# JonasGeiping/fullbatchtraining

Measured on AMD Instinct MI355X. Metric: full-batch GD images/sec (ResNet-18 CIFAR-10 shaped, all chunks accumulated per step), higher is better.
Workload: dtype bf16

## Files before the change

fullbatchtraining_amd/csrc/conv_igemm.hip:

```cpp
#include "common.h"
#include "profile.h"

#include "conv_params.h"

template <typename T, int BN_CO>
__global__ __launch_bounds__(256) void conv_igemm_kernel(const ConvParams p) {
    constexpr int EB = ET<T>::EB;
    constexpr int BKE = 128 / EB;
    constexpr int WROWS = BN_CO / 32;
    constexpr int FI = BN_CO / 32;
    constexpr int FJ = 4;
    constexpr int TILE_CHUNKS = (128 + BN_CO) * 8;
    __shared__ uint4 lds[2 * TILE_CHUNKS];

    const int tid = threadIdx.x, lane = tid & 63, wave = tid >> 6;
    const int wave_co = wave >> 1, wave_px = wave & 1;
    const int mblk = blockIdx.x, co_blk = blockIdx.y, cls = blockIdx.z;
    const int cpy = (p.os == 2) ? (cls >> 1) : 0, cpx = (p.os == 2) ? (cls & 1) : 0;
    const int chunk = tid & 7, lrow = tid >> 3;

    int a_img[4], a_y[4], a_x[4];
    const int qHW = p.qH * p.qW;
#pragma unroll
    for (int i = 0; i < 4; ++i) {
        const int m = mblk * 128 + lrow + 32 * i;
        if (m < p.M) {
            const int n = m / qHW, rem = m - n * qHW, qy = rem / p.qW, qx = rem - qy * p.qW;
            a_img[i] = n * p.Hs * p.Ws; a_y[i] = qy * p.ss; a_x[i] = qx * p.ss;
        } else {
            a_img[i] = 0; a_y[i] = -(1 << 28); a_x[i] = 0;
        }
    }
    const int first_img = (mblk * 128) / qHW;
    const char* wbase = p.wgt + (long long)(first_img / p.imgs_per_wset) * p.wset_stride_bytes;
    const int taps = p.R * p.S;
    const long long wrow_bytes = (long long)taps * p.Cs * EB;
    const char* wptr[WROWS];
#pragma unroll
    for (int i = 0; i < WROWS; ++i) wptr[i] = wbase + (long long)(co_blk * BN_CO + lrow + 32 * i) * wrow_bytes + chunk * 16;

    auto tap_valid = [&](int t, int& dy, int& dx) -> bool {
        const int r = t / p.S, s = t - r * p.S;
        if (p.mode == 0) { dy = r - p.pad; dx = s - p.pad; return true; }
        if (p.os == 1) { dy = p.pad - r; dx = p.pad - s; return true; }
        const int vy = cpy + p.pad - r, vx = cpx + p.pad - s;
        if ((vy & 1) || (vx & 1)) return false;
        dy = vy >> 1; dx = vx >> 1;
        return true;
    };
    const int kc = (p.Cs + BKE - 1) / BKE;
    int n_valid = 0;
    for (int t = 0; t < taps; ++t) { int dy, dx; n_valid += tap_valid(t, dy, dx) ? 1 : 0; }
    const int n_iter = n_valid * kc;

    uint4 ra[4], rw[WROWS];
    int cur_t = -1, cur_c = kc, cur_dy = 0, cur_dx = 0;
    auto advance = [&]() {
        if (++cur_c >= kc) {
            cur_c = 0;
            do { ++cur_t; } while (cur_t < taps && !tap_valid(cur_t, cur_dy, cur_dx));
        }
    };
    auto gload = [&]() {
        const int c0 = cur_c * BKE;
        const bool cvalid = c0 + chunk * ET<T>::VEC < p.Cs;
#pragma unroll
        for (int i = 0; i < 4; ++i) {
            const int sy = a_y[i] + cur_dy, sx = a_x[i] + cur_dx;
            const bool ok = cvalid && (unsigned)sy < (unsigned)p.Hs && (unsigned)sx < (unsigned)p.Ws;
            ra[i] = make_uint4(0, 0, 0, 0);
            if (ok) ra[i] = *(const uint4*)(p.src + ((long long)(a_img[i] + sy * p.Ws + sx) * p.Cs + c0) * EB + chunk * 16);
        }
#pragma unroll
        for (int i = 0; i < WROWS; ++i) {
            rw[i] = make_uint4(0, 0, 0, 0);
            if (cvalid) rw[i] = *(const uint4*)(wptr[i] + ((long long)cur_t * p.Cs + c0) * EB);
        }
    };
    auto lstore = [&](int buf) {
        uint4* base = lds + buf * TILE_CHUNKS;
#pragma unroll
        for (int i = 0; i < 4; ++i) { const int row = lrow + 32 * i; base[row * 8 + (chunk ^ (row & 7))] = ra[i]; }
#pragma unroll
        for (int i = 0; i < WROWS; ++i) { const int row = 128 + lrow + 32 * i; base[row * 8 + (chunk ^ (row & 7))] = rw[i]; }
    };

    f32x4_t acc[FI][FJ];
#pragma unroll
    for (int i = 0; i < FI; ++i)
#pragma unroll
        for (int j = 0; j < FJ; ++j) acc[i][j] = (f32x4_t){0.f, 0.f, 0.f, 0.f};

    if (n_iter > 0) {
        advance(); gload(); lstore(0);
        __syncthreads();
        for (int it = 0; it < n_iter; ++it) {
            const int buf = it & 1;
            const bool more = it + 1 < n_iter;
            if (more) { advance(); gload(); }
            const uint4* base = lds + buf * TILE_CHUNKS;
#pragma unroll
            for (int h = 0; h < 2; ++h) {
                const int pc = ((lane >> 4) + 4 * h) ^ (lane & 7);
                uint4 wf[FI], pf[FJ];
#pragma unroll
                for (int i = 0; i < FI; ++i) wf[i] = base[(128 + wave_co * (BN_CO / 2) + i * 16 + (lane & 15)) * 8 + pc];
#pragma unroll
                for (int j = 0; j < FJ; ++j) pf[j] = base[(wave_px * 64 + j * 16 + (lane & 15)) * 8 + pc];
#pragma unroll
                for (int i = 0; i < FI; ++i)
#pragma unroll
                    for (int j = 0; j < FJ; ++j) acc[i][j] = mma_chunk<T>(wf[i], pf[j], acc[i][j]);
            }
            if (more) lstore(buf ^ 1);
            __syncthreads();
        }
    }

    float ssum[FI][4], ssq[FI][4];
#pragma unroll
    for (int i = 0; i < FI; ++i)
#pragma unroll
        for (int r = 0; r < 4; ++r) { ssum[i][r] = 0.f; ssq[i][r] = 0.f; }
#pragma unroll
    for (int j = 0; j < FJ; ++j) {
        const int m = mblk * 128 + wave_px * 64 + j * 16 + (lane & 15);
        if (m < p.M) {
            const int n = m / qHW, rem = m - n * qHW, qy = rem / p.qW, qx = rem - qy * p.qW;
            const int oy = qy * p.os + cpy, ox = qx * p.os + cpx;
            const long long pix = ((long long)n * p.Hd + oy) * p.Wd + ox;
#pragma unroll
            for (int i = 0; i < FI; ++i) {
                const int co = co_blk * BN_CO + wave_co * (BN_CO / 2) + i * 16 + (lane >> 4) * 4;
                float v[4] = {acc[i][j][0], acc[i][j][1], acc[i][j][2], acc[i][j][3]};
                if (p.addend_mode == 1) {
                    const char* ap = p.addend + (pix * p.Cd + co) * EB;
                    if constexpr (EB == 4) { const float4 a = *(const float4*)ap; v[0] += a.x; v[1] += a.y; v[2] += a.z; v[3] += a.w; }
                    else { const uint2 a = *(const uint2*)ap; v[0] += __uint_as_float(a.x << 16); v[1] += __uint_as_float(a.x & 0xffff0000u);
                           v[2] += __uint_as_float(a.y << 16); v[3] += __uint_as_float(a.y & 0xffff0000u); }
                } else if (p.addend_mode == 2) {
                    const long long apix = ((long long)n * (p.Hd >> 1) + (oy >> 1)) * (p.Wd >> 1) + (ox >> 1);
                    const char* ap = p.addend + (apix * p.Cd + co) * EB;
                    if constexpr (EB == 4) { const float4 a = *(const float4*)ap; v[0] += 0.25f * a.x; v[1] += 0.25f * a.y; v[2] += 0.25f * a.z; v[3] += 0.25f * a.w; }
                    else { const uint2 a = *(const uint2*)ap; v[0] += 0.25f * __uint_as_float(a.x << 16); v[1] += 0.25f * __uint_as_float(a.x & 0xffff0000u);
                           v[2] += 0.25f * __uint_as_float(a.y << 16); v[3] += 0.25f * __uint_as_float(a.y & 0xffff0000u); }
                }
                char* dp = p.dst + (pix * p.Cd + co) * EB;
                if constexpr (EB == 4) *(float4*)dp = make_float4(v[0], v[1], v[2], v[3]);
                else *(uint2*)dp = make_uint2(pack_bf16x2(v[0], v[1]), pack_bf16x2(v[2], v[3]));
#pragma unroll
                for (int r = 0; r < 4; ++r) { ssum[i][r] += v[r]; ssq[i][r] += v[r] * v[r]; }
            }
        }
    }
    if (p.stat != nullptr) {
        float* red = (float*)lds;
        __syncthreads();
#pragma unroll
        for (int i = 0; i < FI; ++i)
#pragma unroll
            for (int r = 0; r < 4; ++r) {
                float a = ssum[i][r], b = ssq[i][r];
                a = row16_sum(a); b = row16_sum(b);
                if ((lane & 15) == 0) {
                    const int col = wave_co * (BN_CO / 2) + i * 16 + (lane >> 4) * 4 + r;
                    red[(wave_px * BN_CO + col) * 2] = a; red[(wave_px * BN_CO + col) * 2 + 1] = b;
                }
            }
        __syncthreads();
        if (tid < BN_CO) {
            const float a = red[tid * 2] + red[(BN_CO + tid) * 2];
            const float b = red[tid * 2 + 1] + red[(BN_CO + tid) * 2 + 1];
            const long long blk = (long long)cls * gridDim.x + mblk;
            p.stat[blk * p.Cd + co_blk * BN_CO + tid] = a;
            p.stat[((long long)p.n_mblocks + blk) * p.Cd + co_blk * BN_CO + tid] = b;
        }
    }
}

int fb_try_conv3x3_halo4(const fb_conv_args* a, hipStream_t st);
int fb_try_conv3x3_halo5(const fb_conv_args* a, hipStream_t st);
int fb_conv3x3_halo5_takes(const fb_conv_args* a);
int fb_try_conv3x3s2_dgrad_quad(const fb_conv_args* a, hipStream_t st);
int fb_try_conv1x1_k32(const fb_conv_args* a, hipStream_t st);
int fb_try_conv1x1_stream(const fb_conv_args* a, hipStream_t st);
int fb_try_conv1x1_gemm(const fb_conv_args* a, hipStream_t st);
int fb_try_conv1x1_pipe(const fb_conv_args* a, hipStream_t st);

int fb_conv1x1_pipe_takes(const fb_conv_args* a);
int fb_conv3x3_halo4_takes(const fb_conv_args* a);
int fb_conv1x1_gemm_takes(const fb_conv_args* a);
static int igemm_masked_addend_ok(const fb_conv_args* a) {
    if (getenv("FB_IGEMM_NO_MASK") != nullptr || a->mode != 1 || a->stride != 1 || a->bst_x) return 0;
    if (a->Cs % 32 != 0 || a->Cd % 64 != 0) return 0;
    static const bool v1 = getenv("FB_IGEMM_V1") != nullptr;
    if (v1) return 0;
    ConvParams p{};
    p.n_img = a->n_img; p.Hs = a->Hs; p.Ws = a->Ws; p.Cs = a->Cs; p.Hd = a->Hd; p.Wd = a->Wd; p.Cd = a->Cd; p.R = a->R; p.S = a->S;
    p.qH = a->Hd; p.qW = a->Wd;
    return fb_igemm_glds_fits(p, a->dtype);
}
extern "C" int32_t fb_conv_masked_addend_supported(const fb_conv_args* a) {
    if (!a || !a->addend || !a->addend_mask || a->addend_mode != 1) return 0;
    return fb_conv3x3_halo5_takes(a) || fb_conv1x1_pipe_takes(a) || fb_conv3x3_halo4_takes(a) || fb_conv1x1_gemm_takes(a) || igemm_masked_addend_ok(a);
}

extern "C" int32_t fb_conv_bwd_stat_supported(const fb_conv_args* a) {
    static const bool disabled = getenv("FB_DISABLE_FUSED_BWD_STAT") != nullptr;
    if (disabled || !a || !a->bst_x || !a->bst_mask || !a->stat_partial || a->mode != 1 || a->dtype != FB_BF16) return 0;
    if ((long long)a->n_img * a->Hd * a->Wd % 128 != 0) return 0;
    static const char* widths = getenv("FB_FUSED_BWD_STAT_W");
    if (widths) {
        char tag[8];
        snprintf(tag, sizeof(tag), "%d,", a->Wd);
        char list[64];
        snprintf(list, sizeof(list), "%s,", widths);
        if (!strstr(list, tag) || (a->Wd < 10 && list != strstr(list, tag) && *(strstr(list, tag) - 1) != ',')) return 0;
    }
    return fb_conv3x3_halo5_takes(a) || fb_conv3x3_halo4_takes(a);
}

template <typename T> static int launch_conv(const ConvParams& p, int classes, hipStream_t st) {
    const int mblocks = (p.M + 127) / 128;
    if (p.Cd % 128 == 0 && (long long)mblocks * (p.Cd / 128) * classes >= 512) {
        dim3 grid(mblocks, p.Cd / 128, classes);
        hipLaunchKernelGGL((conv_igemm_kernel<T, 128>), grid, dim3(256), 0, st, p);
    } else {
        dim3 grid(mblocks, p.Cd / 64, classes);
        hipLaunchKernelGGL((conv_igemm_kernel<T, 64>), grid, dim3(256), 0, st, p);
    }
    return 0;
}

extern "C" int fb_conv2d(const fb_conv_args* a, void* stream) {
    if (!a || !a->src || !a->wgt || !a->dst) FB_FAIL(FB_ERR_ARG, "fb_conv2d: null pointer");
    const int EB = a->dtype == FB_F32 ? 4 : 2;
    if (a->Cs % 32 != 0) FB_FAIL(FB_ERR_SHAPE, "fb_conv2d: Cs=%d must be a multiple of 32", a->Cs);
    if (a->Cd % 64 != 0) FB_FAIL(FB_ERR_SHAPE, "fb_conv2d: Cd=%d must be a multiple of 64", a->Cd);
    if (a->mode != 0 && a->mode != 1) FB_FAIL(FB_ERR_ARG, "fb_conv2d: mode %d", a->mode);
    if (a->addend_mask && !fb_conv_masked_addend_supported(a))
        FB_FAIL(FB_ERR_UNSUPPORTED, "fb_conv2d: addend_mask is not implemented for this shape (ask fb_conv_masked_addend_supported)");
    if (a->bst_x && !fb_conv_bwd_stat_supported(a))
        FB_FAIL(FB_ERR_UNSUPPORTED, "fb_conv2d: the fused BatchNorm-backward reduction is not implemented for this shape (ask fb_conv_bwd_stat_supported)");
    if (a->stride != 1 && a->stride != 2) FB_FAIL(FB_ERR_UNSUPPORTED, "fb_conv2d: stride %d", a->stride);
    ConvParams p;
    p.src = (const char*)a->src; p.wgt = (const char*)a->wgt; p.dst = (char*)a->dst; p.addend = (const char*)a->addend;
    p.stat = a->stat_partial;
    p.n_img = a->n_img; p.Hs = a->Hs; p.Ws = a->Ws; p.Cs = a->Cs; p.Hd = a->Hd; p.Wd = a->Wd; p.Cd = a->Cd;
    p.R = a->R; p.S = a->S; p.stride = a->stride; p.pad = a->pad; p.mode = a->mode;
    p.imgs_per_wset = a->imgs_per_wset > 0 ? a->imgs_per_wset : a->n_img;
    p.wset_stride_bytes = a->wset_stride * EB;
    p.addend_mode = a->addend ? a->addend_mode : 0;
    p.addend_mask = a->addend ? (const unsigned char*)a->addend_mask : nullptr;
    p.amax_src = a->dtype == FB_F32 ? a->amax_src : nullptr; p.amax_wgt = a->dtype == FB_F32 ? a->amax_wgt : nullptr;
    if ((p.amax_src == nullptr) != (p.amax_wgt == nullptr)) FB_FAIL(FB_ERR_ARG, "fb_conv2d: amax_src and amax_wgt go together");
    p.amax_imgs = a->amax_imgs > 0 ? a->amax_imgs : a->n_img;
    int classes = 1;
    if (a->mode == 0) {
        if (a->Hd != (a->Hs + 2 * a->pad - a->R) / a->stride + 1 || a->Wd != (a->Ws + 2 * a->pad - a->S) / a->stride + 1)
            FB_FAIL(FB_ERR_SHAPE, "fb_conv2d: fwd output %dx%d inconsistent with input %dx%d", a->Hd, a->Wd, a->Hs, a->Ws);
        p.qH = a->Hd; p.qW = a->Wd; p.os = 1; p.ss = a->stride;
    } else {
        if (a->Hs != (a->Hd + 2 * a->pad - a->R) / a->stride + 1 || a->Ws != (a->Wd + 2 * a->pad - a->S) / a->stride + 1)
            FB_FAIL(FB_ERR_SHAPE, "fb_conv2d: dgrad shapes inconsistent");
        if (a->stat_partial && !a->bst_x) FB_FAIL(FB_ERR_ARG, "fb_conv2d: statistics in mode 1 need bst_x / bst_mask");
        if (a->stride == 1) { p.qH = a->Hd; p.qW = a->Wd; p.os = 1; }
        else {
            if ((a->Hd & 1) || (a->Wd & 1)) FB_FAIL(FB_ERR_SHAPE, "fb_conv2d: stride-2 dgrad needs even input dims");
            p.qH = a->Hd / 2; p.qW = a->Wd / 2; p.os = 2; classes = 4;
        }
        p.ss = 1;
    }
    p.M = a->n_img * p.qH * p.qW;
    p.n_mblocks = ((p.M + 127) / 128) * classes;
    hipStream_t st = (hipStream_t)stream;
    const int32_t info[FB_PROF_INFO] = {a->n_img, a->Hs, a->Ws, a->Cs, a->Hd, a->Wd, a->Cd, a->R, a->stride,
                                        (a->addend ? a->addend_mode : 0) | (a->addend_mask ? 4 : 0) | (a->bst_x ? 8 : 0) | (a->dtype << 4), 0};
    const int prof = fb_prof_begin(a->mode == 0 ? FB_PROF_IGEMM_FWD : FB_PROF_IGEMM_DGRAD, st, info);
    static const bool v1 = getenv("FB_IGEMM_V1") != nullptr;
    int kernel = 0;
    if (fb_try_conv1x1_k32(a, st)) kernel = FB_K_CONV1X1_K32;
    else if ((a->mode == 0 || a->addend) && (a->Cs == 256 || a->Cs == 128) && fb_try_conv1x1_gemm(a, st)) kernel = FB_K_CONV1X1_GEMM;
    else if (fb_try_conv1x1_pipe(a, st)) kernel = FB_K_CONV1X1_PIPE;
    else if (fb_try_conv1x1_stream(a, st)) kernel = FB_K_CONV1X1_STREAM;
    else if (fb_try_conv1x1_gemm(a, st)) kernel = FB_K_CONV1X1_GEMM;
    else if (fb_try_conv3x3s2_dgrad_quad(a, st)) kernel = FB_K_S2_DGRAD_QUAD;
    else if (fb_try_conv3x3_halo5(a, st)) kernel = FB_K_HALO5;
    else if (fb_try_conv3x3_halo4(a, st)) kernel = FB_K_HALO4;
    else {
        p.zeros = nullptr;
        kernel = FB_K_IGEMM_GLDS;
        if (v1 || !fb_launch_igemm_glds(p, classes, a->dtype, st)) {
            if (p.addend_mask) FB_FAIL(FB_ERR_UNSUPPORTED, "fb_conv2d: the register-staged implicit GEMM does not apply addend_mask (tensor beyond 2^31 bytes per tile or FB_IGEMM_V1)");
            if (p.amax_src) FB_FAIL(FB_ERR_UNSUPPORTED, "fb_conv2d: the register-staged implicit GEMM has no fp16x2 path (tensor beyond 2^31 bytes or FB_IGEMM_V1)");
            if (a->dtype == FB_F32) launch_conv<float>(p, classes, st); else launch_conv<bf16_tag>(p, classes, st);
            kernel = FB_K_IGEMM_V1;
        }
    }
    fb_prof_kernel(prof, kernel);
    fb_prof_end(prof, st);
    FB_CHECK_LAUNCH("fb_conv2d");
    return FB_OK;
}
```

fullbatchtraining_amd/lib.py:

```python
import ctypes as C
import os
import struct

import torch

FB_F32, FB_BF16 = 0, 1
EXPECTED_ABI = 17
_LIB_PATH = os.environ.get("FB_LIB_PATH") or os.path.join(os.path.dirname(os.path.abspath(__file__)), "csrc", "libfbengine.so")

c_void_p, c_int, c_i64, c_float, c_double = C.c_void_p, C.c_int32, C.c_int64, C.c_float, C.c_double


class ConvArgs(C.Structure):
    _fields_ = [("src", c_void_p), ("wgt", c_void_p), ("dst", c_void_p), ("addend", c_void_p), ("stat_partial", c_void_p),
                ("n_img", c_int), ("Hs", c_int), ("Ws", c_int), ("Cs", c_int), ("Hd", c_int), ("Wd", c_int), ("Cd", c_int),
                ("R", c_int), ("S", c_int), ("stride", c_int), ("pad", c_int), ("mode", c_int),
                ("imgs_per_wset", c_int), ("wset_stride", c_i64), ("addend_mode", c_int), ("dtype", c_int), ("addend_mask", c_void_p),
                ("bst_x", c_void_p), ("bst_mask", c_void_p), ("amax_src", c_void_p), ("amax_wgt", c_void_p), ("amax_imgs", c_int)]


class WgradArgs(C.Structure):
    _fields_ = [("x", c_void_p), ("dy", c_void_p), ("dw_partial", c_void_p),
                ("n_img", c_int), ("Hs", c_int), ("Ws", c_int), ("Cs", c_int), ("Hd", c_int), ("Wd", c_int), ("Cd", c_int),
                ("R", c_int), ("S", c_int), ("stride", c_int), ("pad", c_int),
                ("imgs_per_group", c_int), ("split_k", c_int), ("dtype", c_int), ("group_stride", c_i64), ("amax_x", c_void_p), ("amax_dy", c_void_p),
                ("bn_x", c_void_p), ("bn_mask", c_void_p), ("bn_coef", c_void_p)]


_CTYPES = {"v": None, "i": c_int, "l": c_i64, "f": c_float, "d": c_double, "p": c_void_p, "s": C.c_char_p,
           "C": C.POINTER(ConvArgs), "W": C.POINTER(WgradArgs)}
PROF_CLASSES = ("igemm_fwd", "igemm_dgrad", "wgrad", "bn_apply", "bn_bwd_reduce", "bn_bwd_apply")
PROF_KERNELS = {0: "?", 1: "conv_igemm_kernel (register-staged)", 2: "conv_igemm_v3_kernel", 3: "conv3x3s1_halo4_kernel", 4: "conv3x3s1_c64_halo5_kernel",
                5: "conv3x3s2_dgrad_quad_kernel", 6: "conv1x1_k32_kernel", 7: "conv1x1_stream_kernel", 8: "conv3x3s2_fwd_kernel", 9: "conv1x1_pipe_kernel", 10: "conv1x1_gemm_kernel",
                16: "conv_wgrad_kernel", 17: "conv_wgrad3x3_kernel", 18: "conv_wgrad3x3_v2_kernel", 19: "conv_wgrad1x1_kernel"}
_FROM_LIBRARY = ("EXPORTS", "_SIGS", "_ARG_CODES", "MT_BLOCKS", "PROF_INFO")


def __getattr__(name):
    if name in _FROM_LIBRARY:
        load()
        return globals()[name]
    raise AttributeError(f"module {__name__!r} has no attribute {name!r}")


def profile_enable(on, capacity=32768):
    lib = load()
    if lib.fb_profile_enable(1 if on else 0, capacity) != 0:
        raise EngineError(lib.fb_last_error_string().decode())


def profile_read():
    lib = load()
    k = len(PROF_CLASSES)
    ms, n, d = (c_double * k)(), (c_i64 * k)(), (c_i64 * k)()
    if lib.fb_profile_read(ms, n, d) != 0:
        raise EngineError(lib.fb_last_error_string().decode())
    return {k: (ms[i], n[i], d[i]) for i, k in enumerate(PROF_CLASSES)}


def profile_read_launches(cap=1 << 18):
    lib = load()
    info, ms = (c_int * (cap * (PROF_INFO + 1)))(), (c_float * cap)()
    n = lib.fb_profile_read_launches(info, ms, cap)
    if n < 0:
        raise EngineError(lib.fb_last_error_string().decode())
    w = PROF_INFO + 1
    return [(PROF_CLASSES[info[i * w]], tuple(info[i * w + 1:(i + 1) * w]), ms[i]) for i in range(n)]


_lib = None


class EngineError(RuntimeError):
    pass


def check_layout(cls, fields, size):
    mine, end = cls._fields_, 0
    for i, (name, offset, nbytes, code) in enumerate(fields):
        if offset != -(-end // nbytes) * nbytes:
            raise EngineError(f"{cls.__name__}: the library's field {name} at offset {offset} does not follow its predecessor, which ends at {end}")
        end = offset + nbytes
        if i >= len(mine) or mine[i][0] != name:
            raise EngineError(f"{cls.__name__}: field {i} is {name} in the library, {mine[i][0] if i < len(mine) else 'missing'} here")
        here = getattr(cls, name)
        if (here.offset, here.size) != (offset, nbytes) or mine[i][1] is not _CTYPES[code]:
            raise EngineError(f"{cls.__name__}.{name}: {mine[i][1].__name__} of {here.size} bytes at offset {here.offset} here, "
                              f"'{code}' of {nbytes} bytes at offset {offset} in the library")
    if len(mine) > len(fields):
        raise EngineError(f"{cls.__name__}: field {mine[len(fields)][0]} is not in the library's struct")
    if C.sizeof(cls) != size:
        raise EngineError(f"{cls.__name__}: {C.sizeof(cls)} bytes here, {size} in the library")


def _struct_fields(lib, which):
    name, offset, nbytes, code = C.c_char_p(), c_int(), c_int(), C.c_char()
    out = []
    while len(out) < lib.fb_struct_field(which, len(out), C.byref(name), C.byref(offset), C.byref(nbytes), C.byref(code)):
        out.append((name.value.decode(), offset.value, nbytes.value, code.value.decode()))
    return out


def load():
    global _lib, EXPORTS, _SIGS, _ARG_CODES, MT_BLOCKS, PROF_INFO
    if _lib is None:
        if not os.path.isfile(_LIB_PATH):
            raise EngineError(f"{_LIB_PATH} is missing: run `python -m fullbatchtraining_amd.build` (needs hipcc). "
                              "The engine has no CPU or PyTorch fallback.")
        lib = C.CDLL(_LIB_PATH)
        if lib.fb_abi_version() != EXPECTED_ABI:
            raise EngineError(f"{_LIB_PATH} has ABI version {lib.fb_abi_version()}, this package expects {EXPECTED_ABI}: rebuild it with "
                              "`python -m fullbatchtraining_amd.build --force`")
        lib.fb_entry_name.restype = lib.fb_entry_sig.restype = C.c_char_p
        exports, sigs, codes = [], {}, {}
        for i in range(lib.fb_entry_count()):
            name, sig = lib.fb_entry_name(i).decode(), lib.fb_entry_sig(i).decode()
            fn, argtypes = getattr(lib, name), [_CTYPES[c] for c in sig[2:]]
            fn.restype, fn.argtypes = _CTYPES[sig[0]], argtypes
            exports.append(name)
            if lib.fb_entry_kind(i) > 0:
                sigs[name], codes[name] = argtypes, sig[2:]
        for which, cls in enumerate((ConvArgs, WgradArgs)):
            check_layout(cls, _struct_fields(lib, which), lib.fb_struct_size(which))
        if lib.fb_abi_constant(b"FB_PROF_CLASSES") != len(PROF_CLASSES):
            raise EngineError(f"the library times {lib.fb_abi_constant(b'FB_PROF_CLASSES')} kernel classes, PROF_CLASSES names {len(PROF_CLASSES)}")
        EXPORTS, _SIGS, _ARG_CODES = tuple(exports), sigs, codes
        MT_BLOCKS, PROF_INFO = lib.fb_abi_constant(b"FB_MT_BLOCKS"), lib.fb_abi_constant(b"FB_PROF_INFO")
        _lib = lib
    return _lib


def _ptr(t):
    if t is None:
        return None
    if isinstance(t, int):
        return t
    return t.data_ptr()


def _stream():
    return torch.cuda.current_stream().cuda_stream


def call(name, *args):
    lib = load()
    st = _stream()
    status = getattr(lib, name)(*args, st)
    if status != 0:
        raise EngineError(f"{name} failed ({status}): {lib.fb_last_error_string().decode()} [args: {args}]")
    if _recorder is not None:
        _recorder.add_call(name, args, st)


_recorder = None


def recording():
    return _recorder is not None


def current_recorder():
    return _recorder


def _check(status, what):
    if status != 0:
        raise EngineError(f"{what} failed ({status}): {load().fb_last_error_string().decode()}")


def event_new():
    ev = load().fb_event_new()
    if ev < 0:
        raise EngineError(load().fb_last_error_string().decode())
    return ev


def event_count():
    return int(load().fb_event_count())


def event_record(ev, stream=None):
    st = _stream() if stream is None else stream.cuda_stream
    _check(load().fb_event_record(ev, st), "fb_event_record")
    if _recorder is not None:
        _recorder.add_event(1, ev, st)


def event_wait(ev, stream=None):
    st = _stream() if stream is None else stream.cuda_stream
    _check(load().fb_event_wait(ev, st), "fb_event_wait")
    if _recorder is not None:
        _recorder.add_event(2, ev, st)


def _pack_words(name, args):
    load()
    sig = _ARG_CODES[name][:-1]
    if len(args) != len(sig):
        raise EngineError(f"{name}: {len(args)} arguments for a signature of {len(sig)}")
    words = (C.c_uint64 * len(sig))()
    blob = None
    for i, (code, a) in enumerate(zip(sig, args)):
        if code == "f":
            words[i] = struct.unpack("<I", struct.pack("<f", float(a)))[0]
        elif code == "d":
            words[i] = struct.unpack("<Q", struct.pack("<d", float(a)))[0]
        elif code in "pil":
            words[i] = (0 if a is None else int(a)) & 0xFFFFFFFFFFFFFFFF
        elif i == 0 and code in "CW" and hasattr(a, "_obj"):
            blob = a._obj
        else:
            raise EngineError(f"{name}: argument {i} of type '{code}' cannot be recorded")
    return words, blob


class CommandList:

    def __init__(self, handle, n_streams, keep, events=()):
        self.handle, self.n_streams, self.keep, self.events = handle, n_streams, keep, list(events)
        self.used_streams = frozenset()

    def __len__(self):
        return int(load().fb_cmdlist_size(self.handle))

    def replay(self, streams):
        if any(s is None and i in self.used_streams for i, s in enumerate(streams)):
            raise EngineError("CommandList.replay: the list has commands for a stream index that is None now")
        arr = (c_void_p * self.n_streams)(*[None if s is None else s.cuda_stream for s in streams])
        _check(load().fb_cmdlist_replay(self.handle, arr, self.n_streams), "fb_cmdlist_replay")

    def __del__(self):
        try:
            if self.handle and _lib is not None:
                _lib.fb_cmdlist_destroy(self.handle)
        except Exception:
            pass
        self.handle = None


class Recorder:

    def __init__(self, streams):
        self.streams = list(streams)
        self.handles = [None if s is None else s.cuda_stream for s in self.streams]
        self.handle = load().fb_cmdlist_create()
        self.kept = []
        self.events, self.used = [], set()
        self._fn_ids = {}

    def __enter__(self):
        global _recorder
        if _recorder is not None:
            raise EngineError("Recorder: recordings do not nest")
        _recorder = self
        return self

    def __exit__(self, *exc):
        global _recorder
        _recorder = None
        if exc[0] is not None and self.handle:
            load().fb_cmdlist_destroy(self.handle)
            self.handle = None
        return False

    def _stream_index(self, st):
        try:
            return self.handles.index(st)
        except ValueError:
            raise EngineError("Recorder: a call was issued on a stream the recording does not know") from None

    def keep(self, obj):
        self.kept.append(obj)

    def add_call(self, name, args, st):
        fn = self._fn_ids.get(name)
        if fn is None:
            fn = self._fn_ids[name] = load().fb_cmd_fn_id(name.encode())
            if fn < 0:
                raise EngineError(f"Recorder: {name} cannot be part of a command list")
        words, blob = _pack_words(name, args)
        self.used.add(self._stream_index(st))
        _check(load().fb_cmdlist_add_call(self.handle, fn, words, len(words), self._stream_index(st), C.addressof(blob) if blob is not None else None,
                                          C.sizeof(blob) if blob is not None else 0), "fb_cmdlist_add_call")

    def add_event(self, kind, ev, st):
        self.used.add(self._stream_index(st))
        _check(load().fb_cmdlist_add_event(self.handle, kind, ev, self._stream_index(st)), "fb_cmdlist_add_event")

    def finish(self):
        out = CommandList(self.handle, len(self.streams), self.kept, self.events)
        out.used_streams = frozenset(self.used)
        self.handle = None
        return out


def dtype_code(dtype):
    if dtype == torch.float32:
        return FB_F32
    if dtype == torch.bfloat16:
        return FB_BF16
    raise EngineError(f"unsupported compute dtype {dtype}")


def conv2d(src, wgt, dst, R, S, stride, pad, mode, addend=None, addend_mode=0, stat_partial=None, imgs_per_wset=0, wset_stride=0,
           addend_mask=None, bst_x=None, bst_mask=None, amax_src=None, amax_wgt=None, amax_imgs=0):
    n, hs, ws, cs = src.shape
    _, hd, wd, cd = dst.shape
    a = ConvArgs(_ptr(src), _ptr(wgt), _ptr(dst), _ptr(addend), _ptr(stat_partial), n, hs, ws, cs, hd, wd, cd, R, S, stride, pad, mode,
                 imgs_per_wset, wset_stride, addend_mode, dtype_code(src.dtype), _ptr(addend_mask), _ptr(bst_x), _ptr(bst_mask), _ptr(amax_src), _ptr(amax_wgt), amax_imgs)
    if bst_x is not None and not load().fb_conv_bwd_stat_supported(C.byref(a)):
        raise EngineError("fb_conv2d: fused BatchNorm-backward reduction not supported for these arguments")
    call("fb_conv2d", C.byref(a))


def conv2d_wgrad(x, dy, dw_partial, R, S, stride, pad, imgs_per_group, split_k, group_stride=0, amax_x=None, amax_dy=None):
    n, hs, ws, cs = x.shape
    _, hd, wd, cd = dy.shape
    a = WgradArgs(_ptr(x), _ptr(dy), _ptr(dw_partial), n, hs, ws, cs, hd, wd, cd, R, S, stride, pad, imgs_per_group, split_k,
                  dtype_code(x.dtype), group_stride, _ptr(amax_x), _ptr(amax_dy))
    call("fb_conv2d_wgrad", C.byref(a))


def wgrad_reduce(dw_partial, out, out_group_stride, n_groups, split_k, Cd, taps, Cs_pad, Cs_real):
    call("fb_wgrad_reduce", _ptr(dw_partial), _ptr(out), out_group_stride, n_groups, split_k, Cd, taps, Cs_pad, Cs_real)


def weight_prep(master, wset_stride_in, wset_stride_out, n_wsets, Cout, taps, Cin_real, Cin_pad, w_fwd, w_dgrad, dtype, amax=None):
    call("fb_weight_prep", _ptr(master), wset_stride_in, wset_stride_out, n_wsets, Cout, taps, Cin_real, Cin_pad, _ptr(w_fwd),
         _ptr(w_dgrad), dtype_code(dtype), _ptr(amax))
```

Baseline: 218,500.

## Add persistent halo-tiled kernel for 3x3 stride-2 forward conv 64->128

```diff
diff --git a/fullbatchtraining_amd/csrc/conv3x3s2_fwd.hip b/fullbatchtraining_amd/csrc/conv3x3s2_fwd.hip
--- /dev/null
+++ b/fullbatchtraining_amd/csrc/conv3x3s2_fwd.hip
@@ -0,0 +1,211 @@
+#include "common.h"
+
+#include <stdlib.h>
+#include <type_traits>
+
+struct S2FwdParams {
+    const char* src; const char* wgt; char* dst; float* stat;
+    int n_tiles, n_mblocks;
+};
+
+namespace {
+template <int N> __device__ __forceinline__ void s2_wait_vmcnt() { asm volatile("s_waitcnt vmcnt(%0)" ::"n"(N) : "memory"); }
+template <int N> __device__ __forceinline__ void s2_wait_lgkmcnt() {
+    asm volatile("s_waitcnt lgkmcnt(%0)" ::"n"(N) : "memory");
+    __builtin_amdgcn_sched_barrier(0);
+}
+typedef __attribute__((ext_vector_type(4))) unsigned s2_u32x4;
+typedef __attribute__((ext_vector_type(2))) unsigned s2_u32x2;
+template <int OFF> __device__ __forceinline__ uint4 s2_read16(unsigned byte_addr) {
+    static_assert(OFF >= 0 && OFF < 65536, "ds_read_b128: 16-bit immediate");
+    s2_u32x4 v;
+    asm volatile("ds_read_b128 %0, %1 offset:%2" : "=v"(v) : "v"(byte_addr), "n"(OFF));
+    return make_uint4(v[0], v[1], v[2], v[3]);
+}
+template <int I, int N, typename F> __device__ __forceinline__ void s2_static_for(F&& f) {
+    if constexpr (I < N) { f(std::integral_constant<int, I>{}); s2_static_for<I + 1, N>(f); }
+}
+__device__ __forceinline__ int s2_xcd_remap(int b, int n) {
+    const int q = n >> 3, r = n & 7, xcd = b & 7, slot = b >> 3;
+    return (xcd < r ? xcd * (q + 1) : r * (q + 1) + (xcd - r) * q) + slot;
+}
+constexpr unsigned S2_OOB = 0x80000000u;
+constexpr int S2_W = 32, S2_TH = 8;
+constexpr int S2_HROWS = 2 * S2_TH + 1, S2_PITCH = 33;
+constexpr int S2_SLOTS = S2_HROWS * S2_PITCH;
+constexpr int S2_NGRP = (S2_SLOTS + 7) / 8;
+constexpr int S2_HALO_BYTES = S2_NGRP * 1024;
+constexpr int S2_KH = (S2_NGRP + 3) / 4;
+constexpr int S2_ROW_BYTES = S2_PITCH * 128, S2_HI = 8;
+}
+
+__global__ __launch_bounds__(256) void conv3x3s2_fwd_kernel(const S2FwdParams p) {
+#if defined(__HIP_DEVICE_COMPILE__)
+    __shared__ __attribute__((aligned(16))) char lds[2 * S2_HALO_BYTES + 1024];
+
+    const int tid = threadIdx.x, lane = tid & 63;
+    const int wave = __builtin_amdgcn_readfirstlane(tid >> 6);
+    const int NB = gridDim.x;
+    const int lrow8 = lane >> 3, t = lane & 15, g = lane >> 4;
+    const unsigned lds0 = (unsigned)(size_t)(__attribute__((address_space(3))) char*)lds;
+
+    uint4 wr[9][2][2];
+    {
+        const __amdgpu_buffer_rsrc_t rW = __builtin_amdgcn_make_buffer_rsrc((void*)p.wgt, 0, 128 * 9 * 128, 0x00020000);
+#pragma unroll
+        for (int u = 0; u < 9; ++u)
+#pragma unroll
+            for (int h = 0; h < 2; ++h)
+#pragma unroll
+                for (int i = 0; i < 2; ++i) {
+                    const s2_u32x4 v = __builtin_amdgcn_raw_buffer_load_b128(rW, ((wave * 32 + i * 16 + t) * 9 * 128 + (g + 4 * h) * 16), u * 128, 0);
+                    wr[u][h][i] = make_uint4(v[0], v[1], v[2], v[3]);
+                }
+    }
+    unsigned voffH[S2_KH];
+    unsigned topbits = 0;
+#pragma unroll
+    for (int k = 0; k < S2_KH; ++k) {
+        const int q = (wave + 4 * k) * 8 + lrow8;
+        const int hy = q / S2_PITCH, s = q - hy * S2_PITCH;
+        const int ix = s < 17 ? 2 * s - 1 : 2 * (s - 17);
+        const bool ok = q < S2_SLOTS && ix >= 0;
+        voffH[k] = ok ? (unsigned)((hy * S2_W + ix) * 128 + (((lane & 7) ^ (s & 7)) * 16)) : S2_OOB;
+        topbits |= (hy == 0 ? 1u : 0u) << k;
+    }
+    unsigned pb[3][2];
+#pragma unroll
+    for (int b = 0; b < 3; ++b)
+#pragma unroll
+        for (int h = 0; h < 2; ++h) {
+            const int s = (b == 0 ? 0 : b == 1 ? 17 : 1) + t;
+            pb[b][h] = lds0 + s * 128 + (((g + 4 * h) ^ (s & 7)) * 16);
+        }
+    const int voffS = (t * 128 + wave * 32 + (g & 1) * 16 + (g >> 1) * 8) * 2;
+
+    auto halo_piece = [&](auto kc, int buf, int L, bool live) {
+        constexpr int K = decltype(kc)::value;
+        const int grp = wave + 4 * K;
+        const int n0 = L >> 1, y0 = (L & 1) * S2_TH;
+        const long long origin = ((long long)n0 * S2_W + 2 * y0 - 1) * S2_W * 128;
+        const __amdgpu_buffer_rsrc_t rA = __builtin_amdgcn_make_buffer_rsrc((void*)(p.src + origin), 0, S2_HROWS * S2_W * 128, 0x00020000);
+        const unsigned dead = y0 == 0 ? topbits : 0u;
+        const unsigned v = (((dead >> K) & 1u) || !live) ? S2_OOB : voffH[K];
+        const int dst = grp < S2_NGRP ? buf * S2_HALO_BYTES + grp * 1024 : 2 * S2_HALO_BYTES;
+        __builtin_amdgcn_raw_ptr_buffer_load_lds(rA, (__attribute__((address_space(3))) void*)(lds + dst), 16, v, 0, 0, 0);
+    };
+
+    int L = s2_xcd_remap(blockIdx.x, NB);
+    if (L >= p.n_tiles) return;
+    s2_static_for<0, S2_KH>([&](auto kc) { halo_piece(kc, 0, L, true); });
+
+    int buf = 0;
+    for (;;) {
+        const bool has_next = L + NB < p.n_tiles;
+        s2_wait_vmcnt<0>();
+        __builtin_amdgcn_s_barrier();
+        f32x4_t acc[2][8];
+#pragma unroll
+        for (int i = 0; i < 2; ++i)
+#pragma unroll
+            for (int j = 0; j < 8; ++j) acc[i][j] = (f32x4_t){0.f, 0.f, 0.f, 0.f};
+        unsigned pl[3][2], ph[3][2];
+#pragma unroll
+        for (int b = 0; b < 3; ++b)
+#pragma unroll
+            for (int h = 0; h < 2; ++h) { pl[b][h] = pb[b][h] + buf * S2_HALO_BYTES; ph[b][h] = pl[b][h] + S2_HI * S2_ROW_BYTES; }
+
+        uint4 pf[2][8];
+        auto issue_reads = [&](auto sc) {
+            constexpr int S = decltype(sc)::value, U = S >> 1, H = S & 1, A = U / 3, B = U % 3, SET = S & 1;
+            s2_static_for<0, 8>([&](auto jc) {
+                constexpr int J = decltype(jc)::value, ROW = 2 * J + A;
+                if constexpr (ROW < S2_HI) pf[SET][J] = s2_read16<ROW * S2_ROW_BYTES>(pl[B][H]);
+                else pf[SET][J] = s2_read16<(ROW - S2_HI) * S2_ROW_BYTES>(ph[B][H]);
+            });
+        };
+        issue_reads(std::integral_constant<int, 0>{});
+        s2_static_for<0, 18>([&](auto sc) {
+            constexpr int S = decltype(sc)::value, U = S >> 1, H = S & 1, SET = S & 1;
+            if constexpr (S + 1 < 18) {
+                issue_reads(std::integral_constant<int, S + 1>{});
+                s2_wait_lgkmcnt<8>();
+            } else {
+                s2_wait_lgkmcnt<0>();
+            }
+#pragma unroll
+            for (int i = 0; i < 2; ++i)
+#pragma unroll
+                for (int j = 0; j < 8; ++j) acc[i][j] = mma_chunk<bf16_tag>(wr[U][H][i], pf[SET][j], acc[i][j]);
+            halo_piece(sc, buf ^ 1, has_next ? L + NB : L, has_next);
+        });
+
+        {
+            const __amdgpu_buffer_rsrc_t rD = __builtin_amdgcn_make_buffer_rsrc((void*)(p.dst + (long long)L * 128 * 256), 0, 128 * 256, 0x00020000);
+            float ssum[2][4], ssq[2][4];
+#pragma unroll
+            for (int i = 0; i < 2; ++i)
+#pragma unroll
+                for (int r = 0; r < 4; ++r) { ssum[i][r] = 0.f; ssq[i][r] = 0.f; }
+            s2_static_for<0, 8>([&](auto jc) {
+                constexpr int J = decltype(jc)::value;
+                unsigned pk[2][2];
+#pragma unroll
+                for (int i = 0; i < 2; ++i) {
+                    const float v[4] = {acc[i][J][0], acc[i][J][1], acc[i][J][2], acc[i][J][3]};
+                    pk[i][0] = pack_bf16x2(v[0], v[1]); pk[i][1] = pack_bf16x2(v[2], v[3]);
+#pragma unroll
+                    for (int r = 0; r < 4; ++r) { ssum[i][r] += v[r]; ssq[i][r] += v[r] * v[r]; }
+                }
+                const s2_u32x2 lo = __builtin_amdgcn_permlane16_swap(pk[0][0], pk[1][0], false, false);
+                const s2_u32x2 hi = __builtin_amdgcn_permlane16_swap(pk[0][1], pk[1][1], false, false);
+                const s2_u32x4 outv = {lo[0], hi[0], lo[1], hi[1]};
+                __builtin_amdgcn_raw_buffer_store_b128(outv, rD, voffS, J * 16 * 256, 0);
+                store_b128_guard(outv);
+            });
+            if (p.stat != nullptr) {
+#pragma unroll
+                for (int i = 0; i < 2; ++i)
+#pragma unroll
+                    for (int r = 0; r < 4; ++r) { ssum[i][r] = row16_sum(ssum[i][r]); ssq[i][r] = row16_sum(ssq[i][r]); }
+                if (t == 0) {
+#pragma unroll
+                    for (int i = 0; i < 2; ++i) {
+                        const int co = wave * 32 + i * 16 + g * 4;
+                        *(float4*)(p.stat + (long long)L * 128 + co) = make_float4(ssum[i][0], ssum[i][1], ssum[i][2], ssum[i][3]);
+                        *(float4*)(p.stat + ((long long)p.n_mblocks + L) * 128 + co) = make_float4(ssq[i][0], ssq[i][1], ssq[i][2], ssq[i][3]);
+                    }
+                }
+            }
+        }
+        if (!has_next) break;
+        L += NB;
+        buf ^= 1;
+    }
+    s2_wait_vmcnt<0>();
+#endif
+}
+
+int fb_conv3x3s2_fwd_takes(const fb_conv_args* a) {
+    if (getenv("FB_DISABLE_S2FWD") != nullptr) return 0;
+    if (a->dtype != FB_BF16 || a->mode != 0) return 0;
+    if (a->R != 3 || a->S != 3 || a->stride != 2 || a->pad != 1) return 0;
+    if (a->Hs != 32 || a->Ws != 32 || a->Hd != 16 || a->Wd != 16 || a->Cs != 64 || a->Cd != 128) return 0;
+    if (a->n_img < 1) return 0;
+    if (a->imgs_per_wset > 0 && a->imgs_per_wset < a->n_img) return 0;
+    if (a->addend || a->addend_mask || a->bst_x) return 0;
+    if (getenv("FB_S2FWD_ALL") == nullptr && (long long)a->n_img * 2 < 4LL * fb_persistent_cus()) return 0;
+    return 1;
+}
+
+int fb_try_conv3x3s2_fwd(const fb_conv_args* a, hipStream_t st) {
+    if (!fb_conv3x3s2_fwd_takes(a)) return 0;
+    const int n_cu = fb_persistent_cus();
+    S2FwdParams p;
+    p.src = (const char*)a->src; p.wgt = (const char*)a->wgt; p.dst = (char*)a->dst; p.stat = a->stat_partial;
+    p.n_tiles = a->n_img * 2;
+    p.n_mblocks = p.n_tiles;
+    const dim3 grid(p.n_tiles < n_cu ? p.n_tiles : n_cu);
+    hipLaunchKernelGGL(conv3x3s2_fwd_kernel, grid, dim3(256), 0, st, p);
+    return 1;
+}
diff --git a/fullbatchtraining_amd/csrc/conv_igemm.hip b/fullbatchtraining_amd/csrc/conv_igemm.hip
--- a/fullbatchtraining_amd/csrc/conv_igemm.hip
+++ b/fullbatchtraining_amd/csrc/conv_igemm.hip
@@ -182,6 +182,7 @@
 int fb_try_conv3x3_halo5(const fb_conv_args* a, hipStream_t st);
 int fb_conv3x3_halo5_takes(const fb_conv_args* a);
 int fb_try_conv3x3s2_dgrad_quad(const fb_conv_args* a, hipStream_t st);
+int fb_try_conv3x3s2_fwd(const fb_conv_args* a, hipStream_t st);
 int fb_try_conv1x1_k32(const fb_conv_args* a, hipStream_t st);
 int fb_try_conv1x1_stream(const fb_conv_args* a, hipStream_t st);
 int fb_try_conv1x1_gemm(const fb_conv_args* a, hipStream_t st);
@@ -285,6 +286,7 @@
     else if (fb_try_conv1x1_stream(a, st)) kernel = FB_K_CONV1X1_STREAM;
     else if (fb_try_conv1x1_gemm(a, st)) kernel = FB_K_CONV1X1_GEMM;
     else if (fb_try_conv3x3s2_dgrad_quad(a, st)) kernel = FB_K_S2_DGRAD_QUAD;
+    else if (fb_try_conv3x3s2_fwd(a, st)) kernel = FB_K_S2_FWD;
     else if (fb_try_conv3x3_halo5(a, st)) kernel = FB_K_HALO5;
     else if (fb_try_conv3x3_halo4(a, st)) kernel = FB_K_HALO4;
     else {
```

Measured after the change: 219,000 (median of 4 runs). No clear change (+0.2%).

## Add persistent halo-tiled kernel for stride-2 3x3 forward convolutions

Applied to the files above, without the earlier changes.

```diff
diff --git a/fullbatchtraining_amd/csrc/conv3x3s2_fwd_halo.hip b/fullbatchtraining_amd/csrc/conv3x3s2_fwd_halo.hip
--- /dev/null
+++ b/fullbatchtraining_amd/csrc/conv3x3s2_fwd_halo.hip
@@ -0,0 +1,267 @@
+#include "common.h"
+
+#include <type_traits>
+
+struct S2FParams {
+    const char* src; const char* wgt; char* dst; float* stat;
+    int n_img, Cs, Cd, ct_shift, n_tiles;
+    long long M, n_mblocks;
+};
+
+namespace {
+template <int N> __device__ __forceinline__ void s2f_wait_vmcnt() { asm volatile("s_waitcnt vmcnt(%0)" ::"n"(N) : "memory"); }
+template <int N> __device__ __forceinline__ void s2f_wait_lgkmcnt() {
+    asm volatile("s_waitcnt lgkmcnt(%0)" ::"n"(N) : "memory");
+    __builtin_amdgcn_sched_barrier(0);
+}
+typedef __attribute__((ext_vector_type(4))) unsigned s2f_u32x4;
+typedef __attribute__((ext_vector_type(2))) unsigned s2f_u32x2;
+template <int OFF> __device__ __forceinline__ uint4 s2f_read16(unsigned byte_addr) {
+    s2f_u32x4 v;
+    asm volatile("ds_read_b128 %0, %1 offset:%2" : "=v"(v) : "v"(byte_addr), "n"(OFF));
+    return make_uint4(v[0], v[1], v[2], v[3]);
+}
+template <int I, int N, typename F> __device__ __forceinline__ void s2f_static_for(F&& f) {
+    if constexpr (I < N) { f(std::integral_constant<int, I>{}); s2f_static_for<I + 1, N>(f); }
+}
+__device__ __forceinline__ int s2f_xcd_remap(int b, int n) {
+    const int q = n >> 3, r = n & 7, xcd = b & 7, slot = b >> 3;
+    return (xcd < r ? xcd * (q + 1) : r * (q + 1) + (xcd - r) * q) + slot;
+}
+constexpr int s2f_tap_r(int i) { return i < 3 ? 1 : (i == 3 || i == 5 || i == 6 ? 0 : 2); }
+constexpr int s2f_tap_s(int i) { return i == 0 || i == 3 || i == 4 ? 1 : (i == 1 || i == 5 || i == 7 ? 0 : 2); }
+__device__ __forceinline__ int s2f_key(int cell) { return 2 * ((cell >> 2) & 1); }
+
+constexpr int S2F_PLANE = 16384, S2F_HALO = 4 * S2F_PLANE, S2F_WT = 4096, S2F_RED = 4 * 64 * 2 * 4;
+constexpr int S2F_WOFF = S2F_HALO, S2F_ROFF = S2F_WOFF + 3 * S2F_WT, S2F_ZOFF = S2F_ROFF + S2F_RED, S2F_LDS = S2F_ZOFF + 16;
+static_assert(S2F_LDS <= 80 * 1024, "two workgroups per CU");
+
+struct S2FTile { int pt, ct, n0; };
+}
+
+template <int WO>
+__global__ __launch_bounds__(256) __attribute__((amdgpu_waves_per_eu(2, 2))) void conv3x3s2_fwd_halo_kernel(const S2FParams p) {
+#if defined(__HIP_DEVICE_COMPILE__)
+    constexpr int W = 2 * WO, IMGS = 256 / (WO * WO);
+    __shared__ __attribute__((aligned(16))) char lds[S2F_LDS];
+
+    const int tid = threadIdx.x, lane = tid & 63;
+    const int wave = __builtin_amdgcn_readfirstlane(tid >> 6);
+    const int NB = gridDim.x;
+    const int row_b = p.Cs * 2;
+    const int n_hs = row_b / 64;
+    const int px = lane & 15, g4 = lane >> 4;
+    const unsigned lds0 = (unsigned)(size_t)(__attribute__((address_space(3))) char*)lds;
+
+    const int dma_chunk = ((lane & 3) ^ s2f_key(lane >> 2)) * 16;
+    const unsigned voffW = (unsigned)((wave * 16 + (lane >> 2)) * 9 * row_b + dma_chunk);
+    unsigned voffH[4];
+#pragma unroll
+    for (int t = 0; t < 4; ++t) {
+        const int q = wave * 64 + t * 16 + (lane >> 2);
+        const int img_l = q / (WO * WO), qi = q % (WO * WO), oy = qi / WO, ox = qi % WO;
+        voffH[t] = (unsigned)(((img_l * W + 2 * oy) * W + 2 * ox) * row_b + dma_chunk);
+    }
+    unsigned pa[4];
+#pragma unroll
+    for (int d = 0; d < 4; ++d) {
+        const int c = wave * 64 + px - ((d & 2) ? WO : 0) - (d & 1);
+        pa[d] = (unsigned)((int)lds0 + (d ? S2F_PLANE : 0) + c * 64 + ((g4 ^ s2f_key(c)) * 16));
+    }
+    unsigned m_top = 0, m_left = 0;
+#pragma unroll
+    for (int j = 0; j < 4; ++j) {
+        const int qi = (wave * 64 + j * 16 + px) % (WO * WO);
+        m_top |= (qi / WO == 0 ? 1u : 0u) << j;
+        m_left |= (qi % WO == 0 ? 1u : 0u) << j;
+    }
+    const unsigned m_both = m_top | m_left;
+    const unsigned zaddr = lds0 + S2F_ZOFF;
+    const unsigned wa = lds0 + S2F_WOFF + px * 64 + ((g4 ^ s2f_key(px)) * 16);
+    const int voffT = ((wave * 64 + px) * p.Cd + (g4 & 1) * 16 + (g4 >> 1) * 8) * 2;
+    const unsigned redw = lds0 + S2F_ROFF + (wave * 64 + g4 * 4) * 8;
+    const unsigned redr = lds0 + S2F_ROFF + (((tid / 64) * 2) * 64 + (tid % 64)) * 8;
+    if (tid == 0) {
+        const s2f_u32x4 z = {0u, 0u, 0u, 0u};
+        asm volatile("ds_write_b128 %0, %1" ::"v"(zaddr), "v"(z) : "memory");
+    }
+
+    auto decode = [&](int L) {
+        S2FTile t;
+        t.pt = L >> p.ct_shift;
+        t.ct = L - (t.pt << p.ct_shift);
+        t.n0 = t.pt * IMGS;
+        return t;
+    };
+    auto halo_issue = [&](const S2FTile& t, int hs, auto pc) {
+        constexpr int P = decltype(pc)::value;
+        const int imgs = p.n_img - t.n0 < IMGS ? p.n_img - t.n0 : IMGS;
+        const int soff = ((P >> 1) * W + (P & 1)) * row_b + hs * 64;
+        const __amdgpu_buffer_rsrc_t rA =
+            __builtin_amdgcn_make_buffer_rsrc((void*)(p.src + (long long)t.n0 * W * W * row_b + soff), 0, imgs * W * W * row_b - soff, 0x00020000);
+        s2f_static_for<0, 4>([&](auto tc) {
+            constexpr int T = decltype(tc)::value;
+            __builtin_amdgcn_raw_ptr_buffer_load_lds(rA, (__attribute__((address_space(3))) void*)(lds + P * S2F_PLANE + (wave * 4 + T) * 1024), 16, voffH[T], 0, 0, 0);
+        });
+    };
+    auto wt_issue = [&](int buf, const S2FTile& t, int hs, int tap) {
+        const __amdgpu_buffer_rsrc_t rW = __builtin_amdgcn_make_buffer_rsrc((void*)p.wgt, 0, p.Cd * 9 * row_b, 0x00020000);
+        const int soff = t.ct * 64 * 9 * row_b + tap * row_b + hs * 64;
+        __builtin_amdgcn_raw_ptr_buffer_load_lds(rW, (__attribute__((address_space(3))) void*)(lds + S2F_WOFF + buf * S2F_WT + wave * 1024), 16, voffW, soff, 0, 0);
+    };
+
+    int L = s2f_xcd_remap(blockIdx.x, NB);
+    if (L >= p.n_tiles) return;
+    S2FTile cur = decode(L);
+    s2f_static_for<0, 4>([&](auto pc) { halo_issue(cur, 0, pc); });
+    wt_issue(0, cur, 0, s2f_tap_r(0) * 3 + s2f_tap_s(0));
+    wt_issue(1, cur, 0, s2f_tap_r(1) * 3 + s2f_tap_s(1));
+
+    while (true) {
+        const int Ln = L + NB;
+        const bool has_next = Ln < p.n_tiles;
+        S2FTile nxt = cur;
+        if (has_next) nxt = decode(Ln);
+        s2f_wait_vmcnt<0>();
+        s2f_wait_lgkmcnt<0>();
+        __builtin_amdgcn_s_barrier();
+
+        f32x4_t acc[4][4];
+#pragma unroll
+        for (int i = 0; i < 4; ++i)
+#pragma unroll
+            for (int j = 0; j < 4; ++j) acc[i][j] = (f32x4_t){0.f, 0.f, 0.f, 0.f};
+
+        for (int hs = 0; hs < n_hs; ++hs) {
+            const bool more = hs + 1 < n_hs;
+            const bool ahead = more || has_next;
+            const S2FTile nt = more ? cur : nxt;
+            const int nhs = more ? hs + 1 : 0;
+            s2f_static_for<0, 9>([&](auto uc) {
+                constexpr int U = decltype(uc)::value, R = s2f_tap_r(U), S = s2f_tap_s(U);
+                constexpr int BUF = U % 3, NBUF = (U + 2) % 3;
+                constexpr int PL = (R != 1 ? 2 : 0) + (S != 1 ? 1 : 0), D = (R == 0 ? 2 : 0) + (S == 0 ? 1 : 0);
+                if constexpr (U < 7) wt_issue(NBUF, cur, hs, s2f_tap_r(U + 2) * 3 + s2f_tap_s(U + 2));
+                else if (ahead) wt_issue(NBUF, nt, nhs, s2f_tap_r(U - 7) * 3 + s2f_tap_s(U - 7));
+                uint4 wf[4], pf[4];
+                auto rd_p = [&](auto jc) {
+                    constexpr int J = decltype(jc)::value, IMM = (D ? PL - 1 : PL) * S2F_PLANE + J * 1024;
+                    unsigned a = pa[D];
+                    if constexpr (D != 0) {
+                        const unsigned m = D == 1 ? m_left : (D == 2 ? m_top : m_both);
+                        a = ((m >> J) & 1u) ? zaddr - IMM : a;
+                    }
+                    pf[J] = s2f_read16<IMM>(a);
+                };
+                rd_p(std::integral_constant<int, 0>{});
+                s2f_static_for<0, 4>([&](auto i) { wf[decltype(i)::value] = s2f_read16<BUF * S2F_WT +decltype(i)::value * 1024>(wa); });
+                rd_p(std::integral_constant<int, 1>{});
+                rd_p(std::integral_constant<int, 2>{});
+                rd_p(std::integral_constant<int, 3>{});
+                s2f_static_for<0, 4>([&](auto jc) {
+                    constexpr int J = decltype(jc)::value;
+                    s2f_wait_lgkmcnt<3 - J>();
+#pragma unroll
+                    for (int i = 0; i < 4; ++i) acc[i][J] = mma_chunk<bf16_tag>(wf[i], pf[J], acc[i][J]);
+                });
+                constexpr int INFLIGHT = (U == 0 || U == 1 || U == 3 || U == 5) ? 5 : 1;
+                if (ahead) s2f_wait_vmcnt<INFLIGHT>(); else s2f_wait_vmcnt<0>();
+                __builtin_amdgcn_s_barrier();
+                if constexpr (U == 0 || U == 2 || U == 4 || U == 8) {
+                    if (ahead) halo_issue(nt, nhs, std::integral_constant<int, PL>{});
+                }
+            });
+        }
+
+        const long long pix_left = p.M - (long long)cur.pt * 256;
+        const int tile_px = pix_left < 256 ? (int)pix_left : 256;
+        const __amdgpu_buffer_rsrc_t rsrcD = __builtin_amdgcn_make_buffer_rsrc((void*)(p.dst + ((long long)cur.pt * 256 * p.Cd + cur.ct * 64) * 2), 0,
+                                                                                (tile_px * p.Cd - cur.ct * 64) * 2, 0x00020000);
+        float ssum[4][4], ssq[4][4];
+#pragma unroll
+        for (int i = 0; i < 4; ++i)
+#pragma unroll
+            for (int r = 0; r < 4; ++r) { ssum[i][r] = 0.f; ssq[i][r] = 0.f; }
+        s2f_static_for<0, 4>([&](auto jc) {
+            constexpr int J = decltype(jc)::value;
+            const int voff = voffT + J * 16 * p.Cd * 2;
+            unsigned pk[4][2];
+            s2f_static_for<0, 4>([&](auto ic) {
+                constexpr int I = decltype(ic)::value;
+                const float v[4] = {acc[I][J][0], acc[I][J][1], acc[I][J][2], acc[I][J][3]};
+                pk[I][0] = pack_bf16x2(v[0], v[1]); pk[I][1] = pack_bf16x2(v[2], v[3]);
+                if constexpr ((I & 1) == 1) {
+                    const s2f_u32x2 lo = __builtin_amdgcn_permlane16_swap(pk[I - 1][0], pk[I][0], false, false);
+                    const s2f_u32x2 hi = __builtin_amdgcn_permlane16_swap(pk[I - 1][1], pk[I][1], false, false);
+                    const s2f_u32x4 outv = {lo[0], hi[0], lo[1], hi[1]};
+                    __builtin_amdgcn_raw_buffer_store_b128(outv, rsrcD, voff + (I >> 1) * 32 * 2, 0, 0);
+                    store_b128_guard(outv);
+                }
+#pragma unroll
+                for (int r = 0; r < 4; ++r) { ssum[I][r] += v[r]; ssq[I][r] += v[r] * v[r]; }
+            });
+        });
+        if (p.stat != nullptr) {
+#pragma unroll
+            for (int i = 0; i < 4; ++i)
+#pragma unroll
+                for (int r = 0; r < 4; ++r) { ssum[i][r] = row16_sum(ssum[i][r]); ssq[i][r] = row16_sum(ssq[i][r]); }
+            if (px == 0) {
+                s2f_static_for<0, 16>([&](auto c) {
+                    constexpr int I = decltype(c)::value / 4, R = decltype(c)::value % 4;
+                    const f32x2_t d = {ssum[I][R], ssq[I][R]};
+                    const unsigned wr = redw;
+                    asm volatile("ds_write_b64 %0, %1 offset:%2" ::"v"(wr), "v"(d), "n"((I * 16 + R) * 8) : "memory");
+                });
+            }
+            s2f_wait_lgkmcnt<0>();
+            __builtin_amdgcn_s_barrier();
+            if (tid < 128) {
+                const int half = tid / 64, col = tid % 64;
+                f32x2_t x, y;
+                asm volatile("ds_read_b64 %0, %1" : "=v"(x) : "v"(redr));
+                asm volatile("ds_read_b64 %0, %1 offset:%2" : "=v"(y) : "v"(redr), "n"(64 * 8));
+                s2f_wait_lgkmcnt<0>();
+                const long long blk = 2LL * cur.pt + half;
+                if (blk < p.n_mblocks) {
+                    p.stat[blk * p.Cd + cur.ct * 64 + col] = x[0] + y[0];
+                    p.stat[(p.n_mblocks + blk) * p.Cd + cur.ct * 64 + col] = x[1] + y[1];
+                }
+            }
+        }
+        if (!has_next) break;
+        cur = nxt;
+        L = Ln;
+    }
+#endif
+}
+
+int conv3x3s2_fwd_halo_try(const fb_conv_args* a, hipStream_t st) {
+    static const bool disabled = getenv("FB_DISABLE_S2F") != nullptr;
+    if (disabled) return 0;
+    if (a->mode != 0 || a->R != 3 || a->S != 3 || a->stride != 2 || a->pad != 1 || a->dtype != FB_BF16) return 0;
+    if (a->Hs != a->Ws || (a->Hs & 1) || a->Hd != a->Hs / 2 || a->Wd != a->Ws / 2) return 0;
+    const int WO = a->Wd;
+    if (!((WO == 16 && a->Cs == 64) || (WO == 8 && a->Cs == 128) || (WO == 4 && a->Cs == 256)) || a->Cd != 2 * a->Cs) return 0;
+    if (a->addend || a->addend_mask || a->bst_x) return 0;
+    if (a->wset_stride != 0 && a->imgs_per_wset > 0 && a->imgs_per_wset < a->n_img) return 0;
+    const long long M = (long long)a->n_img * WO * WO;
+    if (a->n_img <= 0 || M >= (1LL << 31)) return 0;
+    S2FParams p;
+    p.src = (const char*)a->src; p.wgt = (const char*)a->wgt; p.dst = (char*)a->dst; p.stat = a->stat_partial;
+    p.n_img = a->n_img; p.Cs = a->Cs; p.Cd = a->Cd;
+    p.M = M; p.n_mblocks = (M + 127) / 128;
+    const int n_ct = a->Cd / 64;
+    p.ct_shift = n_ct == 2 ? 1 : (n_ct == 4 ? 2 : 3);
+    const long long n_tiles = (M + 255) / 256 * n_ct;
+    if (n_tiles >= (1LL << 30)) return 0;
+    p.n_tiles = (int)n_tiles;
+    const int slots = 2 * fb_persistent_cus();
+    const char* force = fb_getenv_experimental("FB_S2F_FORCE");
+    if (!(force && atoi(force) != 0) && (WO != 16 || n_tiles < 4LL * slots)) return 0;
+    dim3 grid(p.n_tiles < slots ? p.n_tiles : slots);
+    if (WO == 16) hipLaunchKernelGGL((conv3x3s2_fwd_halo_kernel<16>), grid, dim3(256), 0, st, p);
+    else if (WO == 8) hipLaunchKernelGGL((conv3x3s2_fwd_halo_kernel<8>), grid, dim3(256), 0, st, p);
+    else hipLaunchKernelGGL((conv3x3s2_fwd_halo_kernel<4>), grid, dim3(256), 0, st, p);
+    return 1;
+}
diff --git a/fullbatchtraining_amd/csrc/conv_igemm.hip b/fullbatchtraining_amd/csrc/conv_igemm.hip
--- a/fullbatchtraining_amd/csrc/conv_igemm.hip
+++ b/fullbatchtraining_amd/csrc/conv_igemm.hip
@@ -182,6 +182,7 @@
 int fb_try_conv3x3_halo5(const fb_conv_args* a, hipStream_t st);
 int fb_conv3x3_halo5_takes(const fb_conv_args* a);
 int fb_try_conv3x3s2_dgrad_quad(const fb_conv_args* a, hipStream_t st);
+int conv3x3s2_fwd_halo_try(const fb_conv_args* a, hipStream_t st);
 int fb_try_conv1x1_k32(const fb_conv_args* a, hipStream_t st);
 int fb_try_conv1x1_stream(const fb_conv_args* a, hipStream_t st);
 int fb_try_conv1x1_gemm(const fb_conv_args* a, hipStream_t st);
@@ -287,6 +288,7 @@
     else if (fb_try_conv3x3s2_dgrad_quad(a, st)) kernel = FB_K_S2_DGRAD_QUAD;
     else if (fb_try_conv3x3_halo5(a, st)) kernel = FB_K_HALO5;
     else if (fb_try_conv3x3_halo4(a, st)) kernel = FB_K_HALO4;
+    else if (conv3x3s2_fwd_halo_try(a, st)) kernel = FB_K_S2_FWD;
     else {
         p.zeros = nullptr;
         kernel = FB_K_IGEMM_GLDS;
diff --git a/fullbatchtraining_amd/lib.py b/fullbatchtraining_amd/lib.py
--- a/fullbatchtraining_amd/lib.py
+++ b/fullbatchtraining_amd/lib.py
@@ -31,7 +31,7 @@
            "C": C.POINTER(ConvArgs), "W": C.POINTER(WgradArgs)}
 PROF_CLASSES = ("igemm_fwd", "igemm_dgrad", "wgrad", "bn_apply", "bn_bwd_reduce", "bn_bwd_apply")
 PROF_KERNELS = {0: "?", 1: "conv_igemm_kernel (register-staged)", 2: "conv_igemm_v3_kernel", 3: "conv3x3s1_halo4_kernel", 4: "conv3x3s1_c64_halo5_kernel",
-                5: "conv3x3s2_dgrad_quad_kernel", 6: "conv1x1_k32_kernel", 7: "conv1x1_stream_kernel", 8: "conv3x3s2_fwd_kernel", 9: "conv1x1_pipe_kernel", 10: "conv1x1_gemm_kernel",
+                5: "conv3x3s2_dgrad_quad_kernel", 6: "conv1x1_k32_kernel", 7: "conv1x1_stream_kernel", 8: "conv3x3s2_fwd_halo_kernel", 9: "conv1x1_pipe_kernel", 10: "conv1x1_gemm_kernel",
                 16: "conv_wgrad_kernel", 17: "conv_wgrad3x3_kernel", 18: "conv_wgrad3x3_v2_kernel", 19: "conv_wgrad1x1_kernel"}
 _FROM_LIBRARY = ("EXPORTS", "_SIGS", "_ARG_CODES", "MT_BLOCKS", "PROF_INFO")
 
```

Measured after the change: 223,700 before, 223,700 after, median of 4. Within noise of the previous version (+0.0%).
